# ClarkResearchGroup/cgs-vmc

Measured on NVIDIA B200. Metric: walker_steps_per_sec, higher is better.
Workload: dtype f32

## Files before the change

### cgs_vmc_b200/csrc/rbm2.cu

```cuda
#include <algorithm>
#include <cstdlib>

#include "rbm2_impl.cuh"

namespace cgsvmc {
namespace rbm2 {
namespace {

inline int round_up(int x, int m) { return (x + m - 1) / m * m; }

__global__ void __launch_bounds__(128)
prep_kernel(Image im, const float* __restrict__ a, const float* __restrict__ a0,
            const float* __restrict__ W, const float* __restrict__ c, float* __restrict__ img) {
  __shared__ float red[4];
  const int tid = threadIdx.x;
  if ((int)blockIdx.x < im.N) {
    const int i = blockIdx.x;
    float rs = 0.f;
    for (int j = tid; j < im.HP; j += 128) {
      const float w = j < im.H ? W[(size_t)i * im.H + j] : 0.f;
      img[im.off_w2 + (size_t)i * im.HP + j] = 2.f * w;
      img[im.off_f + (size_t)i * im.HP + j] = expf(4.f * w);
      img[im.off_g + (size_t)i * im.HP + j] = expf(-4.f * w);
      rs += w;
    }
    rs = warp_sum(rs);
    if ((tid & 31) == 0) red[tid >> 5] = rs;
    __syncthreads();
    if (tid == 0) {
      const float total = (red[0] + red[1]) + (red[2] + red[3]);
      img[im.off_a2 + i] = 2.885390081777927f * (a[i] - total);
      img[im.off_a + i] = a[i];
    }
  } else if (blockIdx.x == gridDim.x - 2) {
    uint8_t* lut = reinterpret_cast<uint8_t*>(img + im.off_lut);
    for (int e = tid; e < 2048; e += 128) lut[e] = lut_entry(e);
  } else if (blockIdx.x == gridDim.x - 1) {
    float mx = 0.f;
    for (int e = tid; e < im.N * im.H; e += 128) mx = fmaxf(mx, fabsf(W[e]));
#pragma unroll
    for (int o = 16; o > 0; o >>= 1) mx = fmaxf(mx, __shfl_xor_sync(CGSVMC_FULL_MASK, mx, o));
    if ((tid & 31) == 0) red[tid >> 5] = mx;
    __syncthreads();
    if (tid == 0) {
      img[im.off_a0 + 1] = fmaxf(fmaxf(red[0], red[1]), fmaxf(red[2], red[3]));
      img[im.off_a0 + 2] = 0.f;
      img[im.off_a0 + 3] = 0.f;
    }
  } else {
    const int j = ((int)blockIdx.x - im.N) * 128 + tid;
    if (j < im.HP) {
      float cs = 0.f;
      if (j < im.H)
        for (int i = 0; i < im.N; ++i) cs += W[(size_t)i * im.H + j];
      img[im.off_base + j] = (j < im.H ? c[j] : 0.f) - cs;
    }
    if ((int)blockIdx.x == im.N) {
      if (tid == 0) img[im.off_a0] = a0[0];
      for (int i = im.N + tid; i < im.NP; i += 128) { img[im.off_a2 + i] = 0.f; img[im.off_a + i] = 0.f; }
    }
  }
}

__global__ void __launch_bounds__(256)
reduce_kernel(const float* __restrict__ partials, int n_cta, int64_t stride, int64_t n_out,
              float* __restrict__ out, const double* __restrict__ stat_partials, int64_t B,
              double* __restrict__ stats, uint64_t* counter, uint64_t advance, double* stats_snapshot) {
  __shared__ float sm[8][32];
  constexpr int U = 19;
  const int col = threadIdx.x & 31, slice = threadIdx.x >> 5;
  const int64_t f = (int64_t)blockIdx.x * 32 + col;
  float s = 0.f;
  if (f < n_out) {
    const float* src = partials + f;
    for (int c0 = slice; c0 < n_cta; c0 += 8 * U) {
      float v[U];
#pragma unroll
      for (int u = 0; u < U; ++u) {
        const int c = c0 + 8 * u;
        v[u] = c < n_cta ? __ldcg(src + (size_t)c * stride) : 0.f;
      }
#pragma unroll
      for (int u = 0; u < U; ++u) s += v[u];
    }
  }
  sm[slice][col] = s;
  __syncthreads();
  if (slice == 0 && f < n_out)
    out[f] += ((sm[0][col] + sm[1][col]) + (sm[2][col] + sm[3][col])) +
              ((sm[4][col] + sm[5][col]) + (sm[6][col] + sm[7][col]));
  if (blockIdx.x == 0 && threadIdx.x < 32 && stat_partials != nullptr) {
    double e = 0.0, e2 = 0.0;
// ... 114 lines not shown
  a->pair_tables.push_back(pt);
  return &a->pair_tables.back();
}

int build_pair_table(cgsvmc_ansatz* a, const cgsvmc_ham* h, const Plan& pl,
                     cgsvmc_ansatz::PairTable* slot, cudaStream_t st) {
  if (slot->valid) return CGSVMC_OK;
  pair_prep_kernel<<<2 * h->n_bonds, 128, 0, st>>>(pl.im, a->tables, h->ij, h->n_bonds, slot->buf);
  slot->valid = true;
  return cuda_fail(cudaGetLastError(), "rbm2 pair prep launch");
}

}
}

using namespace rbm2;

bool rbm2_supported(const cgsvmc_ansatz* a, const cgsvmc_ham* h) {
  Plan pl;
  if (!base_plan(a, 1, &pl, true)) return false;
  const int slots = pl.slots;
  const int nb = h != nullptr ? h->n_bonds : 0;
  if (nb >= 32768) return false;
  return walker_smem_bytes(pl.im, slots, false, h != nullptr, nb, true, true) <= (size_t)a->max_smem_optin;
}

int rbm2_mc_steps(cgsvmc_ansatz* a, uint64_t* packed, int64_t B, int n_steps, uint64_t seed,
                  uint64_t walker0, uint64_t step0, unsigned long long* accept_count,
                  float* log_amp_out, cudaStream_t st) {
  Plan pl;
  if (!base_plan(a, B, &pl, false)) { set_error("rbm2: unsupported ansatz"); return CGSVMC_ERR_UNSUPPORTED; }
  const size_t img_bytes = (size_t)pl.im.total * 4;
  pl.ws = img_bytes + 16 <= (size_t)a->max_smem_optin;
  pl.mc_smem = (pl.ws ? img_bytes : 2048) + 16;
  pl.step0_dev = a->step_counter_dev;
  if (int rc = build_image(a, pl, st)) return rc;
  switch (pl.nw) {
    case 1: return launch_mc_nw1(pl, a->tables, packed, B, n_steps, seed, walker0, step0, accept_count, log_amp_out, st);
    case 2: return launch_mc_nw2(pl, a->tables, packed, B, n_steps, seed, walker0, step0, accept_count, log_amp_out, st);
    default: return launch_mc_nw4(pl, a->tables, packed, B, n_steps, seed, walker0, step0, accept_count, log_amp_out, st);
  }
}

int rbm2_walker(cgsvmc_ansatz* a, const cgsvmc_ham* h, const uint64_t* packed, int64_t B,
                float* e_loc, float* log_amp, float* diag, float* off, bool do_grad,
                const float* weights, int K, float* out, double* stats, cudaStream_t st,
                const Rbm2Sweep* sweep) {
  Plan pl;
  if (!base_plan(a, B, &pl, true)) { set_error("rbm2: unsupported ansatz"); return CGSVMC_ERR_UNSUPPORTED; }
  const bool do_eloc = h != nullptr;
  const bool mc = sweep != nullptr;
  const int slots = pl.slots;
  const int nb = do_eloc ? h->n_bonds : 0;
  pl.ws = walker_smem_bytes(pl.im, slots, true, do_eloc, nb, do_grad, mc) <= (size_t)a->max_smem_optin;
  static const bool pt_off = getenv("CGSVMC_RBM2_NO_PAIR_TABLE") != nullptr;
  pl.pt = !pt_off && do_eloc && pl.ws && pl.lpw == 8 && nb >= 1 && nb < 16384 &&
          walker_smem_bytes(pl.im, slots, true, do_eloc, nb, do_grad, mc, true) <= (size_t)a->max_smem_optin;
  const bool pt_global = !pt_off && do_eloc && !pl.ws && nb >= 1 && nb < 16384;
  cgsvmc_ansatz::PairTable* slot =
      (pl.pt || pt_global) ? pair_slot(a, h, (size_t)2 * nb * pl.im.HP * 4) : nullptr;
  if (slot == nullptr) pl.pt = false;
  pl.walker_smem = walker_smem_bytes(pl.im, slots, pl.ws, do_eloc, nb, do_grad, mc, pl.pt);
  if (pl.walker_smem > (size_t)a->max_smem_optin) {
    set_error("rbm2: problem does not fit in shared memory");
    return CGSVMC_ERR_UNSUPPORTED;
  }
  if (int rc = build_image(a, pl, st)) return rc;
  if (slot != nullptr)
    if (int rc = build_pair_table(a, h, pl, slot, st)) return rc;
  const int64_t P = a->n_params;
  WalkerArgs A;
  memset(&A, 0, sizeof(A));
  A.pair_table = slot != nullptr ? slot->buf : nullptr;
  A.packed = packed; A.B = B; A.wpc = pl.wpc; A.n_batches = pl.n_batches;
  A.do_eloc = do_eloc ? 1 : 0;
  if (do_eloc) { A.bonds_ij = h->ij; A.bonds_jx = h->jx; A.bonds_jz = h->jz; A.n_bonds = h->n_bonds; }
  A.e_loc = e_loc; A.log_amp = log_amp; A.diag = diag; A.off = off;
  A.do_grad = do_grad ? 1 : 0;
  A.weights = weights; A.K = K; A.P = P;
  if (mc) {
    A.packed_rw = const_cast<uint64_t*>(packed);
    A.n_steps = sweep->n_steps; A.seed = sweep->seed; A.walker0 = sweep->walker0;
    A.step0 = sweep->step0; A.step0_dev = a->step_counter_dev; A.accept_count = sweep->accept_count;
  }
  {
    const char* e = getenv("CGSVMC_RBM2_TC_GRAD");
    const bool off = e != nullptr && atoi(e) == 0;
    const int np4 = round_up(pl.im.N + 1, 4), np8 = round_up(pl.im.N + 1, 8);
    A.tc_grad = (!off && pl.pt && do_grad && weights == nullptr && np8 == np4 && 3 * np8 <= 128 &&
                 pl.im.H < pl.im.HP && 3 * pl.im.HP <= 512 && (slots == 64 || slots == 128)) ? 1 : 0;
    if (A.tc_grad && e != nullptr && atoi(e) == 2) A.tc_grad = 2;
    const char* sg = getenv("CGSVMC_RBM2_TC_SEGMENT");
    A.tc_segment = sg != nullptr && atoi(sg) > 0 ? atoi(sg) : 8;
  }
  if (mc) A.configs_f32 = sweep->configs_f32;
  const int n_iters = mc && sweep->n_iters > 1 ? sweep->n_iters : 1;
  A.n_iters = n_iters;
  A.out_stride = n_iters > 1 ? B : 0;
  const char* fuse_env = getenv("CGSVMC_RBM2_FUSED_REDUCE");
  const bool fuse_off = fuse_env != nullptr && atoi(fuse_env) == 0;
  bool fuse = false;
  if (do_grad && !fuse_off && pl.grid <= a->num_sms) {
    int coop = 0;
    cudaDeviceGetAttribute(&coop, cudaDevAttrCooperativeLaunch, a->device);
    const int threads = variant_slots(pl.lpw, pl.kjv, true) / (32 / pl.lpw) * 32;
    fuse = coop != 0 && (size_t)slots * pl.im.HP >= (size_t)(threads / 32) * 96;
  }
  if (fuse && a->grid_sync == nullptr) {
    if (int rc = cuda_fail(cudaMalloc(&a->grid_sync, 128), "grid_sync alloc")) return rc;
    if (int rc = cuda_fail(cudaMemset(a->grid_sync, 0, 128), "grid_sync clear")) return rc;
  }
  if (do_grad) {
    const size_t part_bytes = (size_t)pl.grid * 2 * P * sizeof(float);
    const size_t part_pad = (part_bytes + 15) / 16 * 16;
    if (int rc = ensure_scratch(a, part_pad + (size_t)pl.grid * 2 * sizeof(double))) return rc;
    A.partials = a->scratch;
    A.stat_partials = stats != nullptr
        ? reinterpret_cast<double*>(reinterpret_cast<char*>(a->scratch) + part_pad) : nullptr;
  }
  uint64_t* const step_counter = mc ? sweep->advance_counter : nullptr;
  double* const snapshot = mc ? sweep->stats_snapshot : nullptr;
  if (fuse) {
    A.fuse_reduce = (fuse_env != nullptr && atoi(fuse_env) == 2) ? 2 : 1;
    A.sync = a->grid_sync;
    A.out = out; A.n_out = (int64_t)K * P; A.stats = stats;
    A.counter = step_counter; A.advance = mc ? (uint64_t)sweep->n_steps * (uint64_t)n_iters : 0ull;
    A.stats_snapshot = snapshot;
  }
  int rc;
  switch (pl.nw) {
    case 1: rc = launch_walker_nw1(pl, a->tables, A, st); break;
    case 2: rc = launch_walker_nw2(pl, a->tables, A, st); break;
    default: rc = launch_walker_nw4(pl, a->tables, A, st); break;
  }
  if (rc) return rc;
  if (do_grad && !fuse) {
    const int64_t n_out = (int64_t)K * P;
    const int blocks = (int)((n_out + 31) / 32);
    reduce_kernel<<<blocks, 256, 0, st>>>(A.partials, pl.grid, 2 * P, n_out, out, A.stat_partials, B * n_iters, stats,
                                          step_counter, mc ? (uint64_t)sweep->n_steps * (uint64_t)n_iters : 0ull,
                                          snapshot);
    return cuda_fail(cudaGetLastError(), "rbm2 reduce launch");
  }
  return CGSVMC_OK;
}

}
```

### cgs_vmc_b200/csrc/rbm2_impl.cuh

```cuda
#pragma once
#include <cuda_bf16.h>
#include <cuda_fp16.h>

#include "common.cuh"
#include "internal.h"
#include "rbm2.h"

namespace cgsvmc {
namespace rbm2 {

#ifdef CGSVMC_RBM2_TIMING
#define RBM2_TIMING_MARKS 12
static __device__ unsigned long long g_phase_marks[2][160][RBM2_TIMING_MARKS][2];
#define RBM2_MARK(KERN, K)                                                            \
  do {                                                                                \
    if (threadIdx.x == 0 && blockIdx.x < 160) {                                       \
      unsigned long long gt_;                                                         \
      asm volatile("mov.u64 %0, %%globaltimer;" : "=l"(gt_));                         \
      g_phase_marks[KERN][blockIdx.x][K][0] = gt_;                                    \
      g_phase_marks[KERN][blockIdx.x][K][1] = (unsigned long long)clock64();          \
    }                                                                                 \
  } while (0)
#else
#define RBM2_MARK(KERN, K) do {} while (0)
// ... 167 lines not shown
        const float* row = rows + i * HP;
#pragma unroll
        for (int q = 0; q < KJV; ++q) {
          float v[VW];
          ldv<VW, W2S>(row + 32 * q, v);
#pragma unroll
          for (int c = 0; c < VW; c += 2)
            add2(th[VW * q + c], th[VW * q + c + 1], th[VW * q + c], th[VW * q + c + 1], v[c], v[c + 1]);
        }
      }
    }
  }
  float zpart = 0.f;
#pragma unroll
  for (int k = 0; k < KJ; ++k) {
    const float ax = fabsf(th[k]);
    const float e = ex2_approx(-2.885390081777927f * ax);
    const float r = rcp_approx(1.f + e);
    const float big = r, small = e * r;
    p[k] = th[k] >= 0.f ? big : small;
    m[k] = th[k] >= 0.f ? small : big;
    if (want_z) zpart += fmaf(lg2_approx(1.f + e), 0.6931471805599453f, ax - 0.6931471805599453f);
  }
  if (want_z) {
    for (int i = sub; i < im.N; i += LPW) {
      const float ai = ld1<WS>(t.a + i);
      zpart += spin_bit<NW>(s, i) ? ai : -ai;
    }
  }
  return zpart;
}

template <int LPW, int KJV, bool WS, bool KEEP, bool SAFE = false>
__device__ __forceinline__ float exchange_log2_partial(const Tables& t, int d, int u, int sub,
                                                       const float (&p)[32 / LPW * KJV],
                                                       const float (&m)[32 / LPW * KJV],
                                                       float (&tq)[32 / LPW * KJV]) {
  constexpr int VW = 32 / LPW, KJ = VW * KJV, HP = 32 * KJV;
  const float* fr = t.f + d * HP + VW * sub;
  const float* gr = t.g + u * HP + VW * sub;
  float n[KJ];
#pragma unroll
  for (int q = 0; q < KJV; ++q) {
    float f[VW], g[VW];
    ldv<VW, WS>(fr + 32 * q, f);
    ldv<VW, WS>(gr + 32 * q, g);
#pragma unroll
    for (int c = 0; c < VW; c += 2) {
      const int k = VW * q + c;
      float fg0, fg1;
      mul2(fg0, fg1, f[c], f[c + 1], g[c], g[c + 1]);
      if (KEEP) { tq[k] = fg0; tq[k + 1] = fg1; }
      fma2(n[k], n[k + 1], p[k], p[k + 1], fg0, fg1, m[k], m[k + 1]);
    }
  }
  float lsum = 0.f;
  if (SAFE) {
#pragma unroll
    for (int k = 0; k < KJ; ++k) lsum += lg2_approx(n[k]);
  } else {
#pragma unroll
    for (int k = 0; k < KJ; k += 4) {
      float pr;
      if (k + 3 < KJ) {
        float q0, q1;
        mul2(q0, q1, n[k], n[k + 1], n[k + 2], n[k + 3]);
        pr = q0 * q1;
      } else {
        pr = n[k] * n[k + 1];
      }
      lsum += lg2_approx(pr);
    }
  }
  return lsum;
}

template <int LPW, int KJV, bool WS, bool KEEP>
__device__ __forceinline__ float exchange_log2_ratio(const Tables& t, int d, int u, int sub,
                                                     const float (&p)[32 / LPW * KJV],
                                                     const float (&m)[32 / LPW * KJV],
                                                     float (&tq)[32 / LPW * KJV]) {
  const float lsum = group_sum<LPW>(exchange_log2_partial<LPW, KJV, WS, KEEP>(t, d, u, sub, p, m, tq));
  return lsum + (ld1<WS>(t.a2 + d) - ld1<WS>(t.a2 + u));
}

template <int LPW>
__device__ __forceinline__ void transpose_reduce(float (&part)[LPW], int sub) {
#pragma unroll
  for (int o = LPW / 2; o > 0; o >>= 1) {
    const bool upper = (sub & o) != 0;
#pragma unroll
    for (int i = 0; i < o; ++i) {
      const float send = upper ? part[i] : part[i + o];
      const float keep = upper ? part[i + o] : part[i];
      part[i] = keep + __shfl_xor_sync(CGSVMC_FULL_MASK, send, o);
    }
  }
}

template <int LPW, int KJV, bool WS = true>
__device__ __forceinline__ float pair_log2_partial(const float* __restrict__ row, int sub,
                                                   const float (&p)[32 / LPW * KJV],
                                                   const float (&m)[32 / LPW * KJV]) {
  constexpr int VW = 32 / LPW, KJ = VW * KJV;
  float n[KJ];
#pragma unroll
  for (int q = 0; q < KJV; ++q) {
    float tv[VW];
    ldv<VW, WS>(row + VW * sub + 32 * q, tv);
#pragma unroll
    for (int c = 0; c < VW; c += 2) {
      const int k = VW * q + c;
      fma2(n[k], n[k + 1], p[k], p[k + 1], tv[c], tv[c + 1], m[k], m[k + 1]);
    }
  }
  float lsum = 0.f;
#pragma unroll
  for (int k = 0; k < KJ; k += 4) {
    float pr;
    if (k + 3 < KJ) {
      float q0, q1;
      mul2(q0, q1, n[k], n[k + 1], n[k + 2], n[k + 3]);
      pr = q0 * q1;
    } else {
      pr = n[k] * n[k + 1];
    }
    lsum += lg2_approx(pr);
  }
  return lsum;
}

template <int R, int LPW, int KJV, bool WS>
__device__ __forceinline__ float ratio_round(const Tables& t, const uint32_t* list, const int4* bond_s,
                                             int it0, int cnt, int sub,
                                             const float (&p)[32 / LPW * KJV],
                                             const float (&m)[32 / LPW * KJV],
                                             const float* pair_s = nullptr) {
  constexpr int HP = 32 * KJV;
  float part[R], tdummy[32 / LPW * KJV];
  if (pair_s != nullptr) {
#pragma unroll
    for (int i = 0; i < R; ++i) {
      const uint32_t ent = it0 + i < cnt ? list[it0 + i] : 0u;
      const int row = (int)(((ent >> 16) & 0x7fffu) * 2u + (ent >> 31));
      part[i] = pair_log2_partial<LPW, KJV, WS>(pair_s + (size_t)row * HP, sub, p, m);
    }
  } else {
#pragma unroll
    for (int i = 0; i < R; ++i) {
      const uint32_t ent = it0 + i < cnt ? list[it0 + i] : 0u;
      part[i] = exchange_log2_partial<LPW, KJV, WS, false>(t, (int)(ent & 0xffu), (int)((ent >> 8) & 0xffu),
                                                           sub, p, m, tdummy);
    }
  }
#pragma unroll
  for (int o = LPW / 2; o >= R; o >>= 1) {
#pragma unroll
    for (int i = 0; i < R; ++i) part[i] += __shfl_xor_sync(CGSVMC_FULL_MASK, part[i], o);
  }
  transpose_reduce<R>(part, sub & (R - 1));
  const int it = it0 + (sub & (R - 1));
  const bool mine = it < cnt && sub < R;
  const uint32_t ent = mine ? list[it] : 0u;
  const int dn = (int)(ent & 0xffu), up = (int)((ent >> 8) & 0xffu);
  float total = part[0];
  const uint32_t bad = __ballot_sync(CGSVMC_FULL_MASK, mine && !(fabsf(total) <= 3.0e38f));
// ... 83 lines not shown
#pragma unroll
    for (int o = LPW / 2; o > 0; o >>= 1) res |= __shfl_xor_sync(CGSVMC_FULL_MASK, res, o);
    up = (int)(res & 0xffffu);
    dn = (int)(res >> 16);
  }
};

template <int LPW, int KJV, bool WALKER = false>
struct Geometry {
  static constexpr int VW = 32 / LPW, KJ = VW * KJV, HP = 32 * KJV, WPW = 32 / LPW;
  static constexpr int THREADS = (!WALKER && KJ <= 10) ? 1024 : 512;
  static constexpr int WARPS = THREADS / 32, SLOTS = WARPS * WPW;
};

template <int NW, int LPW, int KJV, bool WS>
__device__ __forceinline__ unsigned int mc_sweep(const Tables& t, const Image& im,
                                                 const SitePicker<NW, LPW>& picker, const uint8_t* lut,
                                                 uint64_t (&s)[NW], float (&p)[32 / LPW * KJV],
                                                 float (&m)[32 / LPW * KJV], int sub, bool valid,
                                                 int n_steps, uint64_t seed, uint64_t walker,
                                                 uint64_t step0) {
  constexpr int KJ = 32 / LPW * KJV;
  float tq[KJ];
  const float wbits = 11.541560327111707f * ld1<WS>(t.a0 + 1);
  const int renorm_window = max(1, min(32, (int)((96.f - wbits) / (wbits + 1e-6f))));
  unsigned int n_acc = 0;
  int n_up = 0;
#pragma unroll
  for (int w = 0; w < NW; ++w) n_up += __popcll(s[w]);
  const int n_dn = im.N - n_up;
  const bool can_move = valid && n_up > 0 && n_dn > 0;
  float lnorm = 0.f;
  int since_norm = 0;
  Philox4 rnd = walker_step_random(seed, walker, step0 + (uint64_t)sub);
  uint32_t r0 = __shfl_sync(CGSVMC_FULL_MASK, rnd.x, 0, LPW);
  uint32_t r1 = __shfl_sync(CGSVMC_FULL_MASK, rnd.y, 0, LPW);
  uint32_t r2 = __shfl_sync(CGSVMC_FULL_MASK, rnd.z, 0, LPW);
  for (int step = 0; step < n_steps; ++step) {
    const int k_up = (int)__umulhi(r0, (uint32_t)n_up);
    const int k_dn = (int)__umulhi(r1, (uint32_t)n_dn);
    const float u_acc = u32_to_unit(r2);
    int up, dn;
    picker.pick(s, k_up, k_dn, lut, up, dn);
    if (!can_move) { up = 0; dn = 0; }
    const float lpart = exchange_log2_partial<LPW, KJV, WS, true>(t, dn, up, sub, p, m, tq);
    const float da2 = ld1<WS>(t.a2 + dn) - ld1<WS>(t.a2 + up);
    {
      const int nxt = step + 1;
      if ((nxt & (LPW - 1)) == 0) rnd = walker_step_random(seed, walker, step0 + (uint64_t)(nxt + sub));
      const int src = nxt & (LPW - 1);
      r0 = __shfl_sync(CGSVMC_FULL_MASK, rnd.x, src, LPW);
      r1 = __shfl_sync(CGSVMC_FULL_MASK, rnd.y, src, LPW);
      r2 = __shfl_sync(CGSVMC_FULL_MASK, rnd.z, src, LPW);
    }
    float lfull = group_sum<LPW>(lpart);
    if (__any_sync(CGSVMC_FULL_MASK, !(fabsf(lfull) <= 3.0e38f))) {
      init_state<NW, LPW, KJV, WS>(t, im, s, sub, p, m, false);
      lnorm = 0.f;
      since_norm = 0;
      lfull = group_sum<LPW>(exchange_log2_partial<LPW, KJV, WS, true, true>(t, dn, up, sub, p, m, tq));
    }
    const float l2 = (lfull - lnorm) + da2;
    const float prob = ex2_approx(2.f * l2);
    if (can_move && prob > u_acc) {
#pragma unroll
      for (int k = 0; k < KJ; k += 2) mul2(p[k], p[k + 1], p[k], p[k + 1], tq[k], tq[k + 1]);
      lnorm = lfull;
      flip_bit<NW>(s, up);
      flip_bit<NW>(s, dn);
      ++n_acc;
    }
    if (++since_norm >= renorm_window || __any_sync(CGSVMC_FULL_MASK, fabsf(lnorm) > 48.f)) {
      since_norm = 0;
      lnorm = 0.f;
#pragma unroll
      for (int k = 0; k < KJ; k += 2) {
        float s0, s1;
        add2(s0, s1, p[k], p[k + 1], m[k], m[k + 1]);
        const float r0 = rcp_approx(s0), r1 = rcp_approx(s1);
        mul2(p[k], p[k + 1], p[k], p[k + 1], r0, r1);
        mul2(m[k], m[k + 1], m[k], m[k + 1], r0, r1);
      }
    }
  }
  return n_acc;
}

template <int NW, int LPW, int KJV, bool WS>
__global__ void __launch_bounds__((Geometry<LPW, KJV>::THREADS), 1)
mc_kernel(Image im, const float* __restrict__ img_g, uint64_t* __restrict__ packed, int64_t B,
          int wpc, int64_t n_batches, int n_steps, uint64_t seed, uint64_t walker0, uint64_t step0,
          const uint64_t* __restrict__ step0_dev, unsigned long long* accept_count,
          float* __restrict__ log_amp_out) {
  using Geo = Geometry<LPW, KJV>;
  RBM2_MARK(0, 0);
  if (step0_dev != nullptr) step0 += *step0_dev;
  constexpr int WPW = Geo::WPW, KJ = Geo::KJ;
  extern __shared__ __align__(16) float smem[];
  float* img_s = smem;
  uint8_t* lut = reinterpret_cast<uint8_t*>(smem + (WS ? im.off_lut : 0));
  uint64_t* bar = reinterpret_cast<uint64_t*>(smem + (WS ? im.total : 512));
  const int lane = threadIdx.x & 31, warp = threadIdx.x >> 5;
  const int sub = lane & (LPW - 1), grp = lane / LPW;
  uint64_t s_first[NW];
  {
    const int64_t b = min((int64_t)blockIdx.x * wpc + min(warp * WPW + grp, wpc - 1), B - 1);
#pragma unroll
    for (int w = 0; w < NW; ++w) s_first[w] = w < im.words ? packed[b * im.words + w] : 0ull;
  }
  if (WS) bulk_load(img_s, img_g, (uint32_t)im.total * 4u, bar);
  else build_lut(lut);
  __syncthreads();
  RBM2_MARK(0, 1);
  const Tables t = tables_at(WS ? img_s : img_g, im);
  SitePicker<NW, LPW> picker;
  picker.setup(im.N, sub);
  unsigned int n_acc = 0;
  for (int64_t batch = blockIdx.x; batch < n_batches; batch += gridDim.x) {
    const int slot = warp * WPW + grp;
    const int64_t b = batch * wpc + slot;
    if (warp * WPW >= wpc || batch * wpc + warp * WPW >= B) continue;
    const bool valid = slot < wpc && b < B;
    const int64_t bb = valid ? b : B - 1;
    uint64_t s[NW];
    if (batch == blockIdx.x && valid) {
#pragma unroll
      for (int w = 0; w < NW; ++w) s[w] = s_first[w];
    } else {
#pragma unroll
      for (int w = 0; w < NW; ++w) s[w] = w < im.words ? packed[bb * im.words + w] : 0ull;
    }
    float p[KJ], m[KJ];
    init_state<NW, LPW, KJV, WS>(t, im, s, sub, p, m, false);
    RBM2_MARK(0, 2);
    n_acc += mc_sweep<NW, LPW, KJV, WS>(t, im, picker, lut, s, p, m, sub, valid, n_steps, seed,
                                        walker0 + (uint64_t)bb, step0);
    RBM2_MARK(0, 3);
    if (valid && sub == 0) {
#pragma unroll
      for (int w = 0; w < NW; ++w) if (w < im.words) packed[b * im.words + w] = s[w];
    }
    if (log_amp_out != nullptr) {
      float z = init_state<NW, LPW, KJV, WS>(t, im, s, sub, p, m, true);
      z = group_sum<LPW>(z) + ld1<WS>(t.a0);
      if (valid && sub == 0) log_amp_out[b] = z;
    }
  }
  if (accept_count != nullptr) {
    unsigned int mine = sub == 0 ? n_acc : 0u;
#pragma unroll
    for (int o = 16; o > 0; o >>= 1) mine += __shfl_xor_sync(CGSVMC_FULL_MASK, mine, o);
    if (lane == 0 && mine) atomicAdd(accept_count, (unsigned long long)mine);
  }
  RBM2_MARK(0, 4);
}

template <int THREADS, int NCOL>
__device__ __noinline__ void tcg_drain(uint32_t tmem, float* stg, int n_groups, float* part, int64_t P, int N, int H,
                                       int NC, float e_center, bool add) {
  constexpr int LD = 20;
  const int lane = threadIdx.x & 31, warp = threadIdx.x >> 5;
  const int NPC = 8 * NC;
  const int grp_floats = (128 + NPC) * LD;
  const int wq = warp & 3, g = warp >> 2;
  const int per = 2 * NPC * 4;
  asm volatile("tcgen05.fence::after_thread_sync;" ::: "memory");
// ... 11 lines not shown
                   : "=r"(R[0]), "=r"(R[1]), "=r"(R[2]), "=r"(R[3]), "=r"(R[4]), "=r"(R[5]), "=r"(R[6]), "=r"(R[7]), \
                     "=r"(R[8]), "=r"(R[9]), "=r"(R[10]), "=r"(R[11]), "=r"(R[12]), "=r"(R[13]), "=r"(R[14]), "=r"(R[15]) \
                   : "r"(ADDR) : "memory")
      RBM2_TMEM_LD16(tbase, q0);
      RBM2_TMEM_LD16(tbase + (uint32_t)NCOL, q1);
      if (wq < 2) RBM2_TMEM_LD16(tbase + (uint32_t)(2 * NCOL), q2);
#undef RBM2_TMEM_LD16
      asm volatile("tcgen05.wait::ld.sync.aligned;" ::: "memory");
#pragma unroll
      for (int c = 0; c < 16; c += 4) {
        float4 v;
        v.x = fmaf(__uint_as_float(q1[c]), 1.f / 2048.f, __uint_as_float(q0[c]));
        v.y = fmaf(__uint_as_float(q1[c + 1]), 1.f / 2048.f, __uint_as_float(q0[c + 1]));
        v.z = fmaf(__uint_as_float(q1[c + 2]), 1.f / 2048.f, __uint_as_float(q0[c + 2]));
        v.w = fmaf(__uint_as_float(q1[c + 3]), 1.f / 2048.f, __uint_as_float(q0[c + 3]));
        *reinterpret_cast<float4*>(sg + mrow * LD + c) = v;
        if (wq < 2 && mrow < NPC)
          *reinterpret_cast<float4*>(sg + (128 + mrow) * LD + c) =
              make_float4(__uint_as_float(q2[c]), __uint_as_float(q2[c + 1]), __uint_as_float(q2[c + 2]),
                          __uint_as_float(q2[c + 3]));
      }
    }
    __syncthreads();
#pragma unroll 1
    for (int e = threadIdx.x; e < n_groups * per; e += THREADS) {
      const int gg = e / per, e1 = e - gg * per;
      const int cc0 = cbase + 16 * gg;
      if (cc0 >= NCOL) continue;
      const float* sg = stg + (size_t)gg * grp_floats;
      const int k = e1 >= NPC * 4 ? 1 : 0, r = e1 - k * NPC * 4;
      const int i = r >> 2, c = (r & 3) * 4;
      if (i > N) continue;
      const float4 s0 = *reinterpret_cast<const float4*>(sg + i * LD + c);
      float v[4] = {s0.x, s0.y, s0.z, s0.w};
      if (k == 1) {
        const float4 p1 = *reinterpret_cast<const float4*>(sg + (NPC + i) * LD + c);
        const float4 p2 = *reinterpret_cast<const float4*>(sg + (2 * NPC + i) * LD + c);
        const float4 p3 = *reinterpret_cast<const float4*>(sg + (128 + i) * LD + c);
        const float a1[4] = {p1.x, p1.y, p1.z, p1.w}, a2[4] = {p2.x, p2.y, p2.z, p2.w},
                    a3[4] = {p3.x, p3.y, p3.z, p3.w};
#pragma unroll
        for (int u = 0; u < 4; ++u)
          v[u] = fmaf(e_center, v[u],
                      fmaf(fmaf(a3[u], 1.f / 2048.f, a2[u]), 1.f / 2048.f, a1[u]) * (1.f / kTcgPrescale));
      }
      float* row_w = part + (size_t)k * P + (size_t)(N + 1) + (size_t)i * H;
#pragma unroll
      for (int u = 0; u < 4; ++u) {
        const int j = cc0 + c + u;
        if (j > H) continue;
        float* dst = j < H ? row_w + j : part + (size_t)k * P + i;
        if (add) atomicAdd(dst, v[u]);
        else *dst = v[u];
      }
    }
    __syncthreads();
  }
  asm volatile("tcgen05.fence::before_thread_sync;" ::: "memory");
  __syncthreads();
  asm volatile("tcgen05.fence::after_thread_sync;" ::: "memory");
}

struct WalkerArgs {
  const uint64_t* packed;
  int64_t B;
  int wpc;
  int64_t n_batches;
  int do_eloc;
  const int2* bonds_ij; const float* bonds_jx; const float* bonds_jz; int n_bonds;
  float* e_loc; float* log_amp; float* diag; float* off;
  int do_grad;
  const float* weights;
  int K;
  float* partials;
  double* stat_partials;
  int64_t P;
  uint64_t* packed_rw;
  int n_steps;
  int n_iters;
  int64_t out_stride;
  uint64_t seed, walker0, step0;
  const uint64_t* step0_dev;
  unsigned long long* accept_count;
  const float* pair_table;
  int tc_grad;
  int tc_segment;
  const float* configs_f32;
  int fuse_reduce;
  unsigned int* sync;
  float* out;
  int64_t n_out;
  double* stats;
  uint64_t* counter;
  uint64_t advance;
  double* stats_snapshot;
};

template <int NW, int LPW>
__device__ __forceinline__ void load_walker(const WalkerArgs& A, const Image& im, int64_t bb, int sub,
                                            int grp, uint64_t (&s)[NW]) {
  if (A.configs_f32 == nullptr) {
#pragma unroll
    for (int w = 0; w < NW; ++w) s[w] = w < im.words ? A.packed[bb * im.words + w] : 0ull;
    return;
  }
#pragma unroll
  for (int w = 0; w < NW; ++w) s[w] = 0ull;
  const float* row = A.configs_f32 + bb * im.N;
  for (int i0 = 0; i0 < im.N; i0 += LPW) {
    const int i = i0 + sub;
    const bool up = i < im.N && row[i] > 0.f;
    const uint32_t vote = __ballot_sync(CGSVMC_FULL_MASK, up);
    const uint64_t gbits = (uint64_t)((vote >> (grp * LPW)) & ((1u << LPW) - 1u));
#pragma unroll
    for (int w = 0; w < NW; ++w)
      if ((i0 >> 6) == w) s[w] |= gbits << (i0 & 63);
  }
}

template <int THREADS>
__device__ __forceinline__ void grid_reduce(const WalkerArgs& A, float* red) {
  constexpr int RG = THREADS / 32;
  constexpr int RU = 10;
  constexpr int CU = 3;
  const int lane = threadIdx.x & 31, warp = threadIdx.x >> 5;
  const int n_cta = (int)gridDim.x;
  __syncthreads();
  if (threadIdx.x == 0) {
    __threadfence();
    atomicAdd(&A.sync[0], 1u);
    unsigned int seen;
    do {
      asm volatile("ld.acquire.gpu.global.u32 %0, [%1];" : "=r"(seen) : "l"(A.sync) : "memory");
    } while (seen < (unsigned int)n_cta);
  }
  __syncthreads();
  const int64_t stride = 2 * A.P;
  const int64_t per = (A.n_out + n_cta - 1) / n_cta;
  const int64_t c0 = (int64_t)blockIdx.x * per, c1 = min(A.n_out, c0 + per);
  for (int64_t cbase = c0; cbase < c1; cbase += 32 * CU) {
    float acc[CU];
#pragma unroll
    for (int u = 0; u < CU; ++u) acc[u] = 0.f;
    for (int r0 = warp; r0 < n_cta; r0 += RG * RU) {
      float v[CU][RU];
#pragma unroll
      for (int u = 0; u < CU; ++u) {
        const int64_t col = cbase + 32 * u + lane;
#pragma unroll
        for (int k = 0; k < RU; ++k) {
          const int r = r0 + RG * k;
          v[u][k] = (col < c1 && r < n_cta) ? __ldcg(A.partials + (size_t)r * stride + col) : 0.f;
        }
      }
#pragma unroll
      for (int u = 0; u < CU; ++u)
#pragma unroll
        for (int k = 0; k < RU; ++k) acc[u] += v[u][k];
    }
#pragma unroll
    for (int u = 0; u < CU; ++u) red[warp * (32 * CU) + 32 * u + lane] = acc[u];
    __syncthreads();
    if (threadIdx.x < 32 * CU) {
      const int64_t col = cbase + threadIdx.x;
      if (col < c1) {
        float total = 0.f;
// ... 285 lines not shown
            piece[g] = (uint32_t)__half_as_ushort(b);
            rem = (rem - __half2float(b)) * 2048.f;
          }
          char* ap = reinterpret_cast<char*>(ws_s);
          for (int ch = sub; ch < 4 * NC; ch += LPW) {
            const int g = ch / NC, c = ch - g * NC;
            const uint32_t mag = g == 0 ? 0x3c00u : g == 1 ? piece[0] : g == 2 ? piece[1] : piece[2];
            uint32_t wds[4] = {0u, 0u, 0u, 0u};
#pragma unroll
            for (int e = 0; e < 8; ++e) {
              const int i = 8 * c + e;
              uint32_t hb = 0u;
              if (i < im.N) hb = spin_bit<NW>(s, i) ? mag : (mag ^ 0x8000u);
              else if (i == im.N) hb = mag;
              wds[e >> 1] |= hb << (16 * (e & 1));
            }
            *reinterpret_cast<uint4*>(ap + ((size_t)ch * SLOTS + slot) * 16) = make_uint4(wds[0], wds[1], wds[2], wds[3]);
          }
        } else {
        float* Trow = T_s + slot * HP + VW * sub;
#pragma unroll
        for (int q = 0; q < KJV; ++q) {
          float v[VW];
#pragma unroll
          for (int c = 0; c < VW; ++c) v[c] = p[VW * q + c] - m[VW * q + c];
          stv<VW>(Trow + 32 * q, v);
        }
        float* wrow = ws_s + (size_t)slot * 2 * NP4;
        for (int i = sub; i < NP4; i += LPW) {
          float sg = 0.f;
          if (i < im.N) sg = spin_bit<NW>(s, i) ? 1.f : -1.f;
          else if (i == im.N) sg = 1.f;
          wrow[i] = w0 * sg;
          wrow[NP4 + i] = w1 * sg;
        }
        }
        if (sub == 0) e_s[slot] = e_val;
      }
      RBM2_MARK(1, 4);
    }
    if (A.do_grad) {
      if (threadIdx.x == 0) *tile_next_s = 0;
      if (tcg) {
        for (int e = threadIdx.x; e < (SLOTS - n_valid) * 4 * NC; e += THREADS) {
          const int ch = e / (SLOTS - n_valid), sl = n_valid + e % (SLOTS - n_valid);
          *reinterpret_cast<uint4*>(reinterpret_cast<char*>(ws_s) + ((size_t)ch * SLOTS + sl) * 16) =
              make_uint4(0u, 0u, 0u, 0u);
        }
        asm volatile("fence.proxy.async.shared::cta;" ::: "memory");
      }
      __syncthreads();
      if (tcg && warp == THREADS / 32 - 1) {
        asm volatile("tcgen05.fence::after_thread_sync;" ::: "memory");
        const uint32_t a_units = smem_u32(ws_s) >> 4, b_units = smem_u32(T_s) >> 4;
        const uint32_t hi = (uint32_t)SLOTS | (1u << 14);
        const uint32_t idesc = (1u << 4) | (1u << 15) | (1u << 16) | ((uint32_t)(NCOL >> 3) << 17) | (8u << 24);
        uint32_t elected = 0;
        asm volatile("{ .reg .pred p; elect.sync _|p, 0xffffffff; selp.u32 %0, 1, 0, p; }" : "=r"(elected));
        if (elected) {
          for (int ks = 0; ks < SLOTS / 16; ++ks) {
            const uint32_t accf = ((batch_no % A.tc_segment) > 0 || ks > 0) ? 1u : 0u;
            const uint64_t a0d = ((uint64_t)hi << 32) | ((a_units + (uint32_t)(16 * ks)) | (8u << 16));
            const uint64_t a3d = ((uint64_t)hi << 32) | ((a_units + (uint32_t)(3 * NC * SLOTS + 16 * ks)) | (8u << 16));
            const uint64_t b1d = ((uint64_t)hi << 32) | ((b_units + (uint32_t)(16 * ks)) | (8u << 16));
            const uint64_t b2d = ((uint64_t)hi << 32) | ((b_units + (uint32_t)(NB * SLOTS + 16 * ks)) | (8u << 16));
            const uint64_t ad[3] = {a0d, a0d, a3d}, bd[3] = {b1d, b2d, b1d};
#pragma unroll
            for (int u = 0; u < 3; ++u)
              asm volatile(
                  "{\n\t.reg .pred p;\n\tsetp.ne.b32 p, %4, 0;\n\t"
                  "tcgen05.mma.cta_group::1.kind::f16 [%0], %1, %2, %3, {%5, %5, %5, %5}, p;\n\t}\n"
                  :
                  : "r"(tmem + (uint32_t)(u * NCOL)), "l"(ad[u]), "l"(bd[u]), "r"(idesc), "r"(accf), "r"(0u)
                  : "memory");
          }
          asm volatile("tcgen05.commit.cta_group::1.mbarrier::arrive::one.shared::cluster.b64 [%0];" ::"r"(
                           smem_u32(mma_bar))
                       : "memory");
        }
        __syncwarp();
      }
    }
    if (MC && warp_on) {
      n_acc += mc_sweep<NW, LPW, KJV, WS>(t, im, picker, lut, s, p, m, sub, valid, A.n_steps, A.seed,
                                          A.walker0 + (uint64_t)bb, mc_step0 + (uint64_t)iter * (uint64_t)A.n_steps);
      if (valid && sub == 0) {
#pragma unroll
        for (int w = 0; w < NW; ++w) if (w < im.words) A.packed_rw[b * im.words + w] = s[w];
      }
      __syncwarp();
      RBM2_MARK(1, 5);
    }
    if (A.do_grad) {
      RBM2_MARK(1, 6);
#pragma unroll
      for (int h2 = 0; h2 < 2; ++h2) {
        const int e = rev + h2 * THREADS;
        if (!tcg && e < 2 * NP4) {
#pragma unroll 4
          for (int sb = 0; sb < n_valid; ++sb) acc_a[h2] += ws_s[(size_t)sb * 2 * NP4 + e];
        }
      }
      if (warp == THREADS / 32 - 1 && A.stat_partials != nullptr) {
        double e1 = 0.0, e2 = 0.0;
        for (int sb = lane; sb < n_valid; sb += 32) {
          const double e = (double)e_s[sb];
          e1 += e;
          e2 += e * e;
        }
        sum_e += warp_sum(e1);
        sum_e2 += warp_sum(e2);
      }
      constexpr int TG = 8, TQ = 32 / TG;
      const int tl = lane & (TG - 1), wg = lane / TG;
      for (;;) {
        if (tcg) break;
        int tile_base = 0;
        if (lane == 0) tile_base = atomicAdd(tile_next_s, TG);
        tile_base = __shfl_sync(CGSVMC_FULL_MASK, tile_base, 0);
        if (tile_base >= n_tiles) break;
        const bool tile_ok = tile_base + tl < n_tiles;
        const int tile = min(tile_base + tl, n_tiles - 1);
        const int rt = tile / CT, ct = tile - rt * CT;
        const int i_own = 4 * rt + wg;
        float old[2][4];
#pragma unroll
        for (int k = 0; k < 2; ++k)
#pragma unroll
          for (int c = 0; c < 4; ++c) {
            old[k][c] = 0.f;
            if (batch_no != 0)
              old[k][c] = __ldcg(part + (size_t)k * A.P + im.N + 1 + (size_t)min(i_own, im.N) * im.H +
                                 min(4 * ct + c, im.H - 1));
          }
        float acc[2][4][4];
#pragma unroll
        for (int k = 0; k < 2; ++k)
#pragma unroll
          for (int r = 0; r < 4; ++r)
#pragma unroll
            for (int c = 0; c < 4; ++c) acc[k][r][c] = 0.f;
#pragma unroll 2
        for (int sb = wg; sb < n_valid; sb += TQ) {
          const float4 T = *reinterpret_cast<const float4*>(T_s + sb * HP + 4 * ct);
          const float4 s0 = *reinterpret_cast<const float4*>(ws_s + (size_t)sb * 2 * NP4 + 4 * rt);
          const float4 s1 = *reinterpret_cast<const float4*>(ws_s + (size_t)sb * 2 * NP4 + NP4 + 4 * rt);
          const float tv[4] = {T.x, T.y, T.z, T.w};
          const float a0v[4] = {s0.x, s0.y, s0.z, s0.w};
          const float a1v[4] = {s1.x, s1.y, s1.z, s1.w};
#pragma unroll
          for (int r = 0; r < 4; ++r)
#pragma unroll
            for (int c = 0; c < 4; ++c) {
              acc[0][r][c] = fmaf(a0v[r], tv[c], acc[0][r][c]);
              acc[1][r][c] = fmaf(a1v[r], tv[c], acc[1][r][c]);
            }
        }
        const bool up1 = (wg & 2) != 0, up0 = (wg & 1) != 0;
        float mine[2][4];
#pragma unroll
        for (int k = 0; k < 2; ++k)
#pragma unroll
          for (int c = 0; c < 4; ++c) {
            float h[2];
#pragma unroll
            for (int rr = 0; rr < 2; ++rr) {
              const float send = up1 ? acc[k][rr][c] : acc[k][rr + 2][c];
              const float keep = up1 ? acc[k][rr + 2][c] : acc[k][rr][c];
// ... 146 lines not shown
```

Baseline: 5.377 billion.

## Add speculative two-step Metropolis sweep evaluating consecutive proposals together

Adds a speculative MC sweep that picks sites for two consecutive proposals and computes both exchange log-ratios in one fused pass over the f/g tables. The second result is used only when no lane in the warp accepted the first step and no renormalisation intervened, otherwise it is discarded. A credit counter falls back to single-step evaluation when speculation keeps failing. The aim is more memory-level and instruction parallelism per step and fewer serialized reductions, at the cost of wasted work whenever a step is accepted. The path is enabled by default via an env flag and only runs on the PT path.

After: 4.711 billion (median of 6 runs). 0.876x the previous value.

```diff
diff --git a/cgs_vmc_b200/csrc/rbm2.cu b/cgs_vmc_b200/csrc/rbm2.cu
--- a/cgs_vmc_b200/csrc/rbm2.cu
+++ b/cgs_vmc_b200/csrc/rbm2.cu
@@ -8,6 +8,11 @@
 namespace {
 
 inline int round_up(int x, int m) { return (x + m - 1) / m * m; }
+
+bool spec_enabled() {
+  const char* e = getenv("CGSVMC_RBM2_SPEC");
+  return e == nullptr || atoi(e) != 0;
+}
 
 __global__ void __launch_bounds__(128)
 prep_kernel(Image im, const float* __restrict__ a, const float* __restrict__ a0,
@@ -288,6 +293,7 @@
     A.packed_rw = const_cast<uint64_t*>(packed);
     A.n_steps = sweep->n_steps; A.seed = sweep->seed; A.walker0 = sweep->walker0;
     A.step0 = sweep->step0; A.step0_dev = a->step_counter_dev; A.accept_count = sweep->accept_count;
+    A.spec = spec_enabled() ? 1 : 0;
   }
   {
     const char* e = getenv("CGSVMC_RBM2_TC_GRAD");
diff --git a/cgs_vmc_b200/csrc/rbm2_impl.cuh b/cgs_vmc_b200/csrc/rbm2_impl.cuh
--- a/cgs_vmc_b200/csrc/rbm2_impl.cuh
+++ b/cgs_vmc_b200/csrc/rbm2_impl.cuh
@@ -273,6 +273,65 @@
                                                      float (&tq)[32 / LPW * KJV]) {
   const float lsum = group_sum<LPW>(exchange_log2_partial<LPW, KJV, WS, KEEP>(t, d, u, sub, p, m, tq));
   return lsum + (ld1<WS>(t.a2 + d) - ld1<WS>(t.a2 + u));
+}
+
+template <int LPW, int KJV, bool WS>
+__device__ __forceinline__ void exchange_log2_partial2(const Tables& t, int d0, int u0, int d1, int u1, int sub,
+                                                       const float (&p)[32 / LPW * KJV],
+                                                       const float (&m)[32 / LPW * KJV], float& l0,
+                                                       float& l1) {
+  constexpr int VW = 32 / LPW, HP = 32 * KJV;
+  static_assert(VW == 4, "one four-term product per chunk");
+  const float* f0 = t.f + d0 * HP + VW * sub;
+  const float* g0 = t.g + u0 * HP + VW * sub;
+  const float* f1 = t.f + d1 * HP + VW * sub;
+  const float* g1 = t.g + u1 * HP + VW * sub;
+  l0 = 0.f;
+  l1 = 0.f;
+#pragma unroll
+  for (int q = 0; q < KJV; ++q) {
+    float fa[VW], ga[VW], fb[VW], gb[VW];
+    ldv<VW, WS>(f0 + 32 * q, fa);
+    ldv<VW, WS>(g0 + 32 * q, ga);
+    ldv<VW, WS>(f1 + 32 * q, fb);
+    ldv<VW, WS>(g1 + 32 * q, gb);
+    const int k = VW * q;
+    float na[VW], nb[VW];
+#pragma unroll
+    for (int c = 0; c < VW; c += 2) {
+      float fg0, fg1;
+      mul2(fg0, fg1, fa[c], fa[c + 1], ga[c], ga[c + 1]);
+      fma2(na[c], na[c + 1], p[k + c], p[k + c + 1], fg0, fg1, m[k + c], m[k + c + 1]);
+      mul2(fg0, fg1, fb[c], fb[c + 1], gb[c], gb[c + 1]);
+      fma2(nb[c], nb[c + 1], p[k + c], p[k + c + 1], fg0, fg1, m[k + c], m[k + c + 1]);
+    }
+    float qa0, qa1, qb0, qb1;
+    mul2(qa0, qa1, na[0], na[1], na[2], na[3]);
+    mul2(qb0, qb1, nb[0], nb[1], nb[2], nb[3]);
+    l0 += lg2_approx(qa0 * qa1);
+    l1 += lg2_approx(qb0 * qb1);
+  }
+}
+
+template <int LPW, int KJV, bool WS>
+__device__ __forceinline__ void scale_by_move(const Tables& t, int d, int u, int sub,
+                                              float (&p)[32 / LPW * KJV]) {
+  constexpr int VW = 32 / LPW, HP = 32 * KJV;
+  const float* fr = t.f + d * HP + VW * sub;
+  const float* gr = t.g + u * HP + VW * sub;
+#pragma unroll
+  for (int q = 0; q < KJV; ++q) {
+    float f[VW], g[VW];
+    ldv<VW, WS>(fr + 32 * q, f);
+    ldv<VW, WS>(gr + 32 * q, g);
+#pragma unroll
+    for (int c = 0; c < VW; c += 2) {
+      const int k = VW * q + c;
+      float fg0, fg1;
+      mul2(fg0, fg1, f[c], f[c + 1], g[c], g[c + 1]);
+      mul2(p[k], p[k + 1], p[k], p[k + 1], fg0, fg1);
+    }
+  }
 }
 
 template <int LPW>
@@ -522,6 +581,136 @@
         mul2(m[k], m[k + 1], m[k], m[k + 1], r0, r1);
       }
     }
+  }
+  return n_acc;
+}
+
+template <bool B>
+struct BoolC { static constexpr bool value = B; };
+
+template <int NW, int LPW, int KJV, bool WS>
+__device__ __forceinline__ unsigned int mc_sweep_spec(const Tables& t, const Image& im,
+                                                      const SitePicker<NW, LPW>& picker, const uint8_t* lut,
+                                                      uint64_t (&s)[NW], float (&p)[32 / LPW * KJV],
+                                                      float (&m)[32 / LPW * KJV], int sub, bool valid,
+                                                      int n_steps, uint64_t seed, uint64_t walker,
+                                                      uint64_t step0) {
+  constexpr int KJ = 32 / LPW * KJV;
+  float tdummy[KJ];
+  const float wbits = 11.541560327111707f * ld1<WS>(t.a0 + 1);
+  const int renorm_window = max(1, min(32, (int)((96.f - wbits) / (wbits + 1e-6f))));
+  unsigned int n_acc = 0;
+  int n_up = 0;
+#pragma unroll
+  for (int w = 0; w < NW; ++w) n_up += __popcll(s[w]);
+  const int n_dn = im.N - n_up;
+  const bool can_move = valid && n_up > 0 && n_dn > 0;
+  float lnorm = 0.f;
+  int since_norm = 0;
+  int grp = 0;
+  Philox4 ra = walker_step_random(seed, walker, step0 + (uint64_t)sub);
+  Philox4 rb = walker_step_random(seed, walker, step0 + (uint64_t)(LPW + sub));
+  auto bcast = [&](int x, uint32_t (&r)[3]) {
+    const bool hi = x >= LPW * (grp + 1);
+    const int src = x & (LPW - 1);
+    r[0] = __shfl_sync(CGSVMC_FULL_MASK, hi ? rb.x : ra.x, src, LPW);
+    r[1] = __shfl_sync(CGSVMC_FULL_MASK, hi ? rb.y : ra.y, src, LPW);
+    r[2] = __shfl_sync(CGSVMC_FULL_MASK, hi ? rb.z : ra.z, src, LPW);
+  };
+  uint32_t r_a[3], r_b[3];
+  bcast(0, r_a);
+  bcast(1, r_b);
+  auto pick_sites = [&](const uint32_t (&r)[3], int& up, int& dn, float& da2) {
+    const int k_up = (int)__umulhi(r[0], (uint32_t)n_up);
+    const int k_dn = (int)__umulhi(r[1], (uint32_t)n_dn);
+    picker.pick(s, k_up, k_dn, lut, up, dn);
+    if (!can_move) { up = 0; dn = 0; }
+    da2 = ld1<WS>(t.a2 + dn) - ld1<WS>(t.a2 + up);
+  };
+  auto commit = [&](float lfull, int up, int dn, float da2, uint32_t r2) {
+    const float l2 = (lfull - lnorm) + da2;
+    const float prob = ex2_approx(2.f * l2);
+    const bool acc = can_move && prob > u32_to_unit(r2);
+    if (acc) {
+      scale_by_move<LPW, KJV, WS>(t, dn, up, sub, p);
+      lnorm = lfull;
+      flip_bit<NW>(s, up);
+      flip_bit<NW>(s, dn);
+      ++n_acc;
+    }
+    if (++since_norm >= renorm_window || __any_sync(CGSVMC_FULL_MASK, fabsf(lnorm) > 48.f)) {
+      since_norm = 0;
+      lnorm = 0.f;
+#pragma unroll
+      for (int k = 0; k < KJ; k += 2) {
+        float s0, s1;
+        add2(s0, s1, p[k], p[k + 1], m[k], m[k + 1]);
+        const float r0 = rcp_approx(s0), r1 = rcp_approx(s1);
+        mul2(p[k], p[k + 1], p[k], p[k + 1], r0, r1);
+        mul2(m[k], m[k + 1], m[k], m[k + 1], r0, r1);
+      }
+    }
+    return acc;
+  };
+  constexpr int kSpecCredit = 4;
+  int credit = kSpecCredit;
+  int step = 0;
+  auto pass = [&](auto two_c) {
+    constexpr bool TWO = decltype(two_c)::value;
+    int up_a, dn_a, up_b = 0, dn_b = 0;
+    float da2_a, da2_b = 0.f, lpart_b = 0.f;
+    float lpart_a;
+    if (TWO) {
+      pick_sites(r_a, up_a, dn_a, da2_a);
+      pick_sites(r_b, up_b, dn_b, da2_b);
+      exchange_log2_partial2<LPW, KJV, WS>(t, dn_a, up_a, dn_b, up_b, sub, p, m, lpart_a, lpart_b);
+    } else {
+      pick_sites(r_a, up_a, dn_a, da2_a);
+      lpart_a = exchange_log2_partial<LPW, KJV, WS, false>(t, dn_a, up_a, sub, p, m, tdummy);
+    }
+    if (step + 3 >= LPW * (grp + 2)) {
+      ++grp;
+      ra = rb;
+      rb = walker_step_random(seed, walker, step0 + (uint64_t)(LPW * (grp + 1) + sub));
+    }
+    uint32_t r_c[3], r_d[3];
+    bcast(step + 2, r_c);
+    if (TWO) bcast(step + 3, r_d);
+    float lfull_a = group_sum<LPW>(lpart_a);
+    const float lfull_b = TWO ? group_sum<LPW>(lpart_b) : 0.f;
+    bool repaired = false;
+    if (__any_sync(CGSVMC_FULL_MASK, !(fabsf(lfull_a) <= 3.0e38f))) {
+      init_state<NW, LPW, KJV, WS>(t, im, s, sub, p, m, false);
+      lnorm = 0.f;
+      since_norm = 0;
+      repaired = true;
+      lfull_a = group_sum<LPW>(exchange_log2_partial<LPW, KJV, WS, false, true>(t, dn_a, up_a, sub, p, m, tdummy));
+    }
+    int adv = 0;
+    float lfull = lfull_a, da2 = da2_a;
+    int up = up_a, dn = dn_a;
+    uint32_t r2 = r_a[2];
+#pragma unroll 1
+    for (;;) {
+      const bool acc = commit(lfull, up, dn, da2, r2);
+      if (++adv == 2) break;
+      const bool two_ok = !repaired && since_norm != 0 &&
+                          !__any_sync(CGSVMC_FULL_MASK, acc || (TWO && !(fabsf(lfull_b) <= 3.0e38f)));
+      credit = two_ok ? min(credit + 1, kSpecCredit) : max(credit - 1, 0);
+      if (!TWO || !two_ok) break;
+      lfull = lfull_b; da2 = da2_b; up = up_b; dn = dn_b; r2 = r_b[2];
+    }
+#pragma unroll
+    for (int i = 0; i < 3; ++i) {
+      const uint32_t c = r_c[i];
+      r_a[i] = adv == 2 ? c : r_b[i];
+      r_b[i] = adv == 2 ? (TWO ? r_d[i] : c) : c;
+    }
+    return adv;
+  };
+  while (step < n_steps) {
+    if (credit > 0 && step + 1 < n_steps) step += pass(BoolC<true>());
+    else step += pass(BoolC<false>());
   }
   return n_acc;
 }
@@ -699,6 +888,7 @@
   uint64_t seed, walker0, step0;
   const uint64_t* step0_dev;
   unsigned long long* accept_count;
+  int spec;
   const float* pair_table;
   int tc_grad;
   int tc_segment;
@@ -1150,8 +1340,18 @@
       }
     }
     if (MC && warp_on) {
-      n_acc += mc_sweep<NW, LPW, KJV, WS>(t, im, picker, lut, s, p, m, sub, valid, A.n_steps, A.seed,
-                                          A.walker0 + (uint64_t)bb, mc_step0 + (uint64_t)iter * (uint64_t)A.n_steps);
+      const uint64_t walker = A.walker0 + (uint64_t)bb, step0 = mc_step0 + (uint64_t)iter * (uint64_t)A.n_steps;
+      bool done = false;
+      if constexpr (PT) {
+        if (A.spec) {
+          n_acc += mc_sweep_spec<NW, LPW, KJV, WS>(t, im, picker, lut, s, p, m, sub, valid, A.n_steps, A.seed,
+                                                   walker, step0);
+          done = true;
+        }
+      }
+      if (!done)
+        n_acc += mc_sweep<NW, LPW, KJV, WS>(t, im, picker, lut, s, p, m, sub, valid, A.n_steps, A.seed,
+                                            walker, step0);
       if (valid && sub == 0) {
 #pragma unroll
         for (int w = 0; w < NW; ++w) if (w < im.words) A.packed_rw[b * im.words + w] = s[w];
```
